# mp3guy/ElasticFusion

Hardware: NVIDIA H100
Metric: frames/sec, full track+fuse+predict (processFrame) (higher is better)
Workload: dtype f32

## Files before the change

elasticfusion_b200/csrc/ef_api.cu:

```cuda
#include <math.h>
#include <stddef.h>
#include <stdio.h>
#include <stdlib.h>
#include <string.h>

#include <new>
#include <utility>
#include <vector>

#include "ef_dmath.cuh"
#include "ef_internal.h"

using namespace ef;

extern "C" void ef_default_config(EfConfig* c, int width, int height, float fx, float fy, float cx, float cy) {
  memset(c, 0, sizeof(*c));
  c->width = width;
  c->height = height;
  c->fx = fx;
  c->fy = fy;
  c->cx = cx;
  c->cy = cy;
  c->time_delta = 200;
  c->count_thresh = 35000;
// ... 23 lines not shown
  if (code > 0) return cudaGetErrorString((cudaError_t)code);
  return "unknown error";
}

static int alloc_odom(EfContext* ctx, OdomDev& od) {
  const EfConfig& c = ctx->cfg;
  memset(&od, 0, sizeof(od));
  od.width = c.width;
  od.height = c.height;
  od.distThres = 0.10f;
  od.angleThres = sinf(20.f * 3.14159254f / 180.f);
  od.sobelScale = (float)(1.0 / pow(2.0, 3));
  od.maxDepthDeltaRGB = 0.07f;
  od.maxDepthRGB = 6.0f;
  od.minGrad[0] = 5;
  od.minGrad[1] = 3;
  od.minGrad[2] = 1;
  for (int i = 0; i < NUM_PYRS; ++i) {
    od.minScale[i] = (float)(pow((double)od.minGrad[i], 2.0) / pow((double)od.sobelScale, 2.0));
    od.rows[i] = c.height >> i;
    od.cols[i] = c.width >> i;
    const size_t n = (size_t)od.rows[i] * od.cols[i];
    CU(ctx_alloc(ctx, &od.depth_tmp[i], n, 0));
    CU(ctx_alloc(ctx, &od.vmap_g_prev[i], 3 * n, 0xff));
    CU(ctx_alloc(ctx, &od.nmap_g_prev[i], 3 * n, 0xff));
    CU(ctx_alloc(ctx, &od.vmap_c_prev[i], 3 * n, 0xff));
    CU(ctx_alloc(ctx, &od.nmap_c_prev[i], 3 * n, 0xff));
    CU(ctx_alloc(ctx, &od.vmap_curr[i], 3 * n, 0xff));
    CU(ctx_alloc(ctx, &od.nmap_curr[i], 3 * n, 0xff));
    CU(ctx_alloc(ctx, &od.lastDepth[i], n, 0xff));
    CU(ctx_alloc(ctx, &od.nextDepth[i], n, 0xff));
    CU(ctx_alloc(ctx, &od.lastImage[i], n, 0));
    CU(ctx_alloc(ctx, &od.nextImage[i], n, 0));
    CU(ctx_alloc(ctx, &od.lastNextImage[i], n, 0));
    CU(ctx_alloc(ctx, &od.dIdx[i], n, 0));
    CU(ctx_alloc(ctx, &od.dIdy[i], n, 0));
    CU(ctx_alloc(ctx, &od.corres[i], n, 0));
  }
  const size_t n0 = (size_t)c.width * c.height;
  CU(ctx_alloc(ctx, &od.vmaps_tmp, 4 * n0, 0));
  CU(ctx_alloc(ctx, &od.gn, 1));
  od.cand_base = reinterpret_cast<const int*>(reinterpret_cast<const char*>(od.gn) + offsetof(GNState, cand_base));
  od.intr0 = reinterpret_cast<const float*>(reinterpret_cast<const char*>(od.gn) + offsetof(GNState, fx));
  od.K_levels = reinterpret_cast<const double*>(reinterpret_cast<const char*>(od.gn) + offsetof(GNState, Kd));
  CU(ctx_alloc(ctx, &od.so3s, 1, 0));
  CU(ctx_alloc(ctx, &od.so3_partials, (size_t)MAX_RED_BLOCKS * PARTIAL_STRIDE, 0));
  CU(ctx_alloc(ctx, &od.so3_counter, 4, 0));
  CU(ctx_alloc(ctx, &od.partials, (size_t)MAX_RED_BLOCKS * PARTIAL_STRIDE, 0));
  CU(ctx_alloc(ctx, &od.partials_rgb, (size_t)MAX_RGB_BLOCKS * 32, 0));
  CU(ctx_alloc(ctx, &od.partials2, (size_t)MAX_RGB_BLOCKS * 32, 0));
  {
    size_t flat = 0;
    for (int i = 0; i < NUM_PYRS; ++i) {
      od.level_start[i] = (int)flat;
      flat += (size_t)od.rows[i] * od.cols[i];
    }
    od.level_start[NUM_PYRS] = (int)flat;
    CU(ctx_alloc(ctx, &od.cand, flat, 0));
    CU(ctx_alloc(ctx, &od.terms, flat, 0));
  }
  CU(ctx_alloc(ctx, &od.partials_i, (size_t)MAX_RED_BLOCKS * 2));
  CU(ctx_alloc(ctx, &od.counter, 4, 0));
  CU(ctx_alloc(ctx, &od.trace, MAX_TRACE, 0));
  GNState g;
  memset(&g, 0, sizeof(g));
  for (int k = 0; k < 16; ++k) g.T_wc[k] = (k % 5 == 0) ? 1.0 : 0.0;
  g.lastICPCount = g.lastRGBCount = g.lastSO3Count = (float)(c.width * c.height);
  g.fx = c.fx;
  g.fy = c.fy;
  g.cx = c.cx;
  g.cy = c.cy;
  for (int lv = 0; lv < NUM_PYRS; ++lv) {
    const int div = 1 << lv;
    const double fx = (double)(c.fx / div), fy = (double)(c.fy / div), cx = (double)(c.cx / div), cy = (double)(c.cy / div);
    const double K[9] = {fx, 0, cx, 0, fy, cy, 0, 0, 1};
    const double ifx = 1.0 / fx, ify = 1.0 / fy;
    const double Ki[9] = {ifx, 0, -cx * ifx, 0, ify, -cy * ify, 0, 0, 1};
    for (int k = 0; k < 9; ++k) {
      g.Kd[lv][k] = K[k];
      g.Kinvd[lv][k] = Ki[k];
    }
  }
  g.break_level = -1;
  g.weighting = 1.0f;
  g.flat_n = od.level_start[NUM_PYRS];
  CU(cudaMemcpyAsync(od.gn, &g, sizeof(g), cudaMemcpyHostToDevice, ctx->stream));
  CU(cudaStreamSynchronize(ctx->stream));
  return 0;
}

static int create_buffers(EfContext* ctx) {
  RC(alloc_odom(ctx, ctx->odom[0]));
  RC(alloc_odom(ctx, ctx->odom[1]));
  const size_t n = (size_t)ctx->cfg.width * ctx->cfg.height;
  Textures& t = ctx->tex;
  memset(&t, 0, sizeof(t));
  CU(ctx_alloc(ctx, &t.rgb, n * 3, 0));
  CU(ctx_alloc(ctx, &t.rgba, n * 4, 0));
  CU(ctx_alloc(ctx, &t.depth_raw, n, 0));
  CU(ctx_alloc(ctx, &t.depth_filtered, n, 0));
  CU(ctx_alloc(ctx, &t.depth_metric, n, 0));
  CU(ctx_alloc(ctx, &t.depth_metric_filtered, n, 0));
  CU(ctx_alloc(ctx, &t.index, n, 0));
  CU(ctx_alloc(ctx, &t.vert_conf, n, 0));
  CU(ctx_alloc(ctx, &t.color_time, n, 0));
  CU(ctx_alloc(ctx, &t.norm_rad, n, 0));
  CU(ctx_alloc(ctx, &t.image, n, 0));
  CU(ctx_alloc(ctx, &t.old_image, n, 0));
  CU(ctx_alloc(ctx, &t.fill_image, n, 0));
  CU(ctx_alloc(ctx, &t.vertex, n, 0));
  CU(ctx_alloc(ctx, &t.normal, n, 0));
  CU(ctx_alloc(ctx, &t.old_vertex, n, 0));
  CU(ctx_alloc(ctx, &t.old_normal, n, 0));
  CU(ctx_alloc(ctx, &t.fill_vertex, n, 0));
  CU(ctx_alloc(ctx, &t.fill_normal, n, 0));
  CU(ctx_alloc(ctx, &t.time, n, 0));
  CU(ctx_alloc(ctx, &t.old_time, n, 0));
  CU(ctx_alloc(ctx, &t.synth_depth, n, 0));
  Lookahead& la = ctx->la;
  memset(&la, 0, sizeof(la));
  CU(ctx_alloc(ctx, &la.rgb, n * 3, 0));
  CU(ctx_alloc(ctx, &la.rgba, n * 4, 0));
  CU(ctx_alloc(ctx, &la.depth_raw, n, 0));
  CU(ctx_alloc(ctx, &la.depth_filtered, n, 0));
  CU(ctx_alloc(ctx, &la.depth_metric, n, 0));
  CU(ctx_alloc(ctx, &la.depth_metric_filtered, n, 0));
  for (int i = 0; i < NUM_PYRS; ++i) {
    const size_t ni = (size_t)ctx->odom[0].rows[i] * ctx->odom[0].cols[i];
    CU(ctx_alloc(ctx, &la.depth_tmp[i], ni, 0));
    CU(ctx_alloc(ctx, &la.vmap_curr[i], 3 * ni, 0xff));
    CU(ctx_alloc(ctx, &la.nmap_curr[i], 3 * ni, 0xff));
    CU(ctx_alloc(ctx, &la.image[i], ni, 0));
  }
  CU(ctx_alloc(ctx, &la.so3s, 1, 0));
  CU(ctx_alloc(ctx, &la.so3_partials, (size_t)MAX_RED_BLOCKS * PARTIAL_STRIDE, 0));
  CU(ctx_alloc(ctx, &la.so3_counter, 4, 0));
  CU(cudaStreamCreateWithFlags(&la.stream, cudaStreamNonBlocking));
  CU(cudaEventCreateWithFlags(&la.ready, cudaEventDisableTiming));
  CU(cudaEventCreateWithFlags(&la.spare_free, cudaEventDisableTiming));
  CU(cudaEventCreateWithFlags(&la.h2d_done, cudaEventDisableTiming));
  CU(cudaEventCreateWithFlags(&la.image_ready, cudaEventDisableTiming));
  CU(cudaEventCreateWithFlags(&la.track_started, cudaEventDisableTiming));
  if (ctx->stage_timing) {
    CU(cudaEventCreate(&la.timing[0]));
    CU(cudaEventCreate(&la.timing[1]));
  }
  CU(cudaMallocHost((void**)&la.pin_rgb, n * 3));
  CU(cudaMallocHost((void**)&la.pin_depth, n * 2));
  RC(alloc_map(ctx));
  CU(cudaMallocHost((void**)&ctx->pin_rgb, n * 3));
  CU(cudaMallocHost((void**)&ctx->pin_depth, n * 2));
  CU(cudaMallocHost((void**)&ctx->pin_small, sizeof(PinStaging)));
  CU(cudaMalloc((void**)&ctx->dev_small, sizeof(DevStaging)));
  CU(cudaEventRecord(la.spare_free, ctx->stream));
  CU(cudaEventRecord(la.h2d_done, la.stream));
  CU(cudaEventRecord(la.image_ready, ctx->stream));
  CU(cudaStreamSynchronize(ctx->stream));
  return 0;
}

extern "C" int ef_create(const EfConfig* cfg, void* stream, EfContext** out) {
  if (!cfg || !out || cfg->width <= 0 || cfg->height <= 0 || cfg->capacity <= 0) return EF_EINVAL;
  if (cfg->reloc) return EF_EINVAL;
  if ((cfg->width >> 2) < 8 || (cfg->height >> 2) < 8) return EF_EINVAL;
  CU(cudaSetDevice(cfg->device));
  EfContext* ctx = new (std::nothrow) EfContext();
  if (!ctx) return EF_ENOMEM;
  ctx->cfg = *cfg;
  ctx->device = cfg->device;
  {
    int sms = 0;
    cudaError_t e = cudaDeviceGetAttribute(&sms, cudaDevAttrMultiProcessorCount, cfg->device);
    ctx->num_sms = sms;
    ctx->own_stream = false;
    if (e == cudaSuccess) {
      if (stream) {
        ctx->stream = (cudaStream_t)stream;
      } else {
        e = cudaStreamCreateWithFlags(&ctx->stream, cudaStreamNonBlocking);
        ctx->own_stream = (e == cudaSuccess);
      }
    }
    if (e != cudaSuccess) {
      delete ctx;
      return (int)e;
    }
  }
  ctx->launches = 0;
  ctx->so3_ready = false;
  {
    const char* e = getenv("EF_NO_PDL");
    ctx->pdl = !(e && e[0] == '1');
    ctx->plain_next = false;
    ctx->maps_dirty[0] = ctx->maps_dirty[1] = true;
    e = getenv("EF_VISIBLE_LIST");
    ctx->visible_list = !(e && e[0] == '0');
    ctx->vis_pending = false;
    e = getenv("EF_GN_CLUSTER");
    ctx->gn_cluster = odom_cluster_size(e ? atoi(e) : 16);
    e = getenv("EF_GN_CLUSTER_LEVELS");
    ctx->gn_cluster_levels = e ? atoi(e) : 1;
    if (ctx->gn_cluster_levels < 0) ctx->gn_cluster_levels = 0;
    if (ctx->gn_cluster_levels > NUM_PYRS) ctx->gn_cluster_levels = NUM_PYRS;
    e = getenv("EF_STAGE_TIMING");
    ctx->stage_timing = (e && e[0] == '1');
    ctx->stage_n = 0;
    if (ctx->stage_timing)
      for (int i = 0; i < 16; ++i) cudaEventCreate(&ctx->stage_ev[i]);
    e = getenv("EF_LA_AFTER_TRACK");
    ctx->la_after_track = !(e && e[0] == '0');
  }
  ctx->tick = 1;
  for (int k = 0; k < 16; ++k) ctx->T_wc[k] = (k % 5 == 0) ? 1.0 : 0.0;
  ctx->rgb_only = false;
  ctx->icp_weight = cfg->icp_weight;
  ctx->pyramid = true;
  ctx->fast_odom = cfg->fast_odom != 0;
  ctx->so3 = cfg->so3 != 0;
  ctx->frame_to_frame_rgb = cfg->frame_to_frame_rgb != 0;
  ctx->confidence = cfg->confidence;
  ctx->depth_cutoff = cfg->depth_cutoff;
  ctx->max_depth_processed = 20.0f;
  ctx->host_count = 0;
  ctx->frame_open = false;

  if (int rc = create_buffers(ctx)) {
    ef_destroy(ctx);
    return rc;
  }
  *out = ctx;
  return 0;
}

extern "C" int ef_destroy(EfContext* ctx) {
  if (!ctx) return EF_EINVAL;
  cudaSetDevice(ctx->device);
  cudaStreamSynchronize(ctx->stream);
  if (ctx->la.stream) {
    cudaStreamSynchronize(ctx->la.stream);
    cudaStreamDestroy(ctx->la.stream);
  }
  if (ctx->la.ready) cudaEventDestroy(ctx->la.ready);
  if (ctx->la.spare_free) cudaEventDestroy(ctx->la.spare_free);
  if (ctx->la.h2d_done) cudaEventDestroy(ctx->la.h2d_done);
  if (ctx->la.image_ready) cudaEventDestroy(ctx->la.image_ready);
  if (ctx->la.track_started) cudaEventDestroy(ctx->la.track_started);
  for (cudaEvent_t ev : ctx->la.timing)
    if (ev) cudaEventDestroy(ev);
  if (ctx->la.pin_rgb) cudaFreeHost(ctx->la.pin_rgb);
  if (ctx->la.pin_depth) cudaFreeHost(ctx->la.pin_depth);
  map_free_host(ctx);
  deform_free(ctx);
  ctx->arena.release();
  if (ctx->pin_rgb) cudaFreeHost(ctx->pin_rgb);
  if (ctx->pin_depth) cudaFreeHost(ctx->pin_depth);
  if (ctx->pin_small) cudaFreeHost(ctx->pin_small);
  if (ctx->dev_small) cudaFree(ctx->dev_small);
  if (ctx->own_stream) cudaStreamDestroy(ctx->stream);
  delete ctx;
  return 0;
}

extern "C" void* ef_stream(EfContext* ctx) { return ctx ? (void*)ctx->stream : nullptr; }
extern "C" int ef_sync(EfContext* ctx) {
  if (!ctx) return EF_EINVAL;
  CU(cudaStreamSynchronize(ctx->stream));
  CU(cudaStreamSynchronize(ctx->la.stream));
  return 0;
}
extern "C" int ef_launch_count(EfContext* ctx, int64_t* n) {
  if (!ctx || !n) return EF_EINVAL;
  *n = ctx->launches;
  return 0;
}

extern "C" int ef_buffer(EfContext* ctx, int32_t id, int32_t level, void** dev_ptr, size_t* bytes) {
  if (!ctx) return EF_EINVAL;
  const size_t n = (size_t)ctx->cfg.width * ctx->cfg.height;
  void* p = nullptr;
  size_t b = 0;
  Textures& t = ctx->tex;
  if (id < 40) {
    switch (id) {
      case EF_BUF_RGB: p = t.rgb; b = n * 3; break;
      case EF_BUF_RGBA: p = t.rgba; b = n * 4; break;
      case EF_BUF_DEPTH_RAW: p = t.depth_raw; b = n * 2; break;
      case EF_BUF_DEPTH_FILTERED: p = t.depth_filtered; b = n * 2; break;
      case EF_BUF_DEPTH_METRIC: p = t.depth_metric; b = n * 4; break;
      case EF_BUF_DEPTH_METRIC_FILTERED: p = t.depth_metric_filtered; b = n * 4; break;
      case EF_BUF_INDEX: p = t.index; b = n * 4; break;
      case EF_BUF_VERT_CONF: p = t.vert_conf; b = n * 16; break;
      case EF_BUF_COLOR_TIME: p = t.color_time; b = n * 16; break;
      case EF_BUF_NORM_RAD: p = t.norm_rad; b = n * 16; break;
      case EF_BUF_IMAGE: p = t.image; b = n * 4; break;
      case EF_BUF_VERTEX: p = t.vertex; b = n * 16; break;
      case EF_BUF_NORMAL: p = t.normal; b = n * 16; break;
      case EF_BUF_TIME: p = t.time; b = n * 2; break;
      case EF_BUF_OLD_IMAGE: p = t.old_image; b = n * 4; break;
      case EF_BUF_OLD_VERTEX: p = t.old_vertex; b = n * 16; break;
      case EF_BUF_OLD_NORMAL: p = t.old_normal; b = n * 16; break;
      case EF_BUF_OLD_TIME: p = t.old_time; b = n * 2; break;
      case EF_BUF_SYNTH_DEPTH: p = t.synth_depth; b = n * 4; break;
      case EF_BUF_FILL_IMAGE: p = t.fill_image; b = n * 4; break;
      case EF_BUF_FILL_VERTEX: p = t.fill_vertex; b = n * 16; break;
      case EF_BUF_FILL_NORMAL: p = t.fill_normal; b = n * 16; break;
      default: return EF_EINVAL;
// ... 535 lines not shown
    ef_stage(ctx, 10);
  }
  if (ctx->tick == 1) RC(map_update_pose_async(ctx, nullptr));
  RC(predict_async(ctx));
  ef_stage(ctx, 11);
  ctx->tick++;
  ctx->frame_open = false;
  return 0;
}

extern "C" int ef_process_frame_device(EfContext* ctx, const uint8_t* rgb_dev, const uint16_t* depth_dev, int64_t timestamp,
                                       float weight_multiplier, const double* in_T_wc) {
  (void)timestamp;
  if (!ctx || ((rgb_dev == nullptr) != (depth_dev == nullptr))) return EF_EINVAL;
  RC(frame_begin_device(ctx, rgb_dev, depth_dev, weight_multiplier, in_T_wc));
  return frame_end_device(ctx, 0, false);
}

static int stage_host_frame(EfContext* ctx, const uint8_t* rgb, const uint16_t* depth) {
  const size_t n = (size_t)ctx->cfg.width * ctx->cfg.height;
  CU(cudaStreamSynchronize(ctx->stream));
  memcpy(ctx->pin_rgb, rgb, n * 3);
  memcpy(ctx->pin_depth, depth, n * 2);
  CU(cudaMemcpyAsync(ctx->tex.rgb, ctx->pin_rgb, n * 3, cudaMemcpyHostToDevice, ctx->stream));
  CU(cudaMemcpyAsync(ctx->tex.depth_raw, ctx->pin_depth, n * 2, cudaMemcpyHostToDevice, ctx->stream));
  return 0;
}

extern "C" int ef_process_frame_begin(EfContext* ctx, const uint8_t* rgb, const uint16_t* depth, int64_t timestamp, float weight_multiplier,
                                      const double* in_T_wc) {
  (void)timestamp;
  if (!ctx || !rgb || !depth) return EF_EINVAL;
  if (ctx->la.pending || ctx->frame_open) return EF_ESTATE;
  RC(stage_host_frame(ctx, rgb, depth));
  RC(frame_begin_device(ctx, ctx->tex.rgb, ctx->tex.depth_raw, weight_multiplier, in_T_wc));
  return ef_finish_frame(ctx);
}

extern "C" int ef_process_frame_end(EfContext* ctx, const double* T_wc_override, const float* graph_nodes16, int32_t n_nodes, int32_t fern_accepted) {
  if (!ctx || n_nodes < 0 || (n_nodes > 0 && !graph_nodes16)) return EF_EINVAL;
  if (!ctx->frame_open) return EF_ESTATE;
  if (T_wc_override) {
    RC(ef_set_pose(ctx, T_wc_override));
    RC(map_update_pose_async(ctx, nullptr));
  }
  RC(map_set_graph(ctx, graph_nodes16, n_nodes));
  RC(frame_end_device(ctx, n_nodes, fern_accepted != 0));
  return ef_finish_frame(ctx);
}

extern "C" int ef_local_loop_result(EfContext* ctx, EfLoopResult* out, double* src3, double* dst3, int32_t* times, int32_t max_constraints,
                                    int32_t* n_out) {
  if (!ctx || !out || max_constraints < 0) return EF_EINVAL;
  const MapDev& m = ctx->map;
  LoopDev h;
  CU(cudaMemcpyAsync(&h, m.loop, sizeof(h), cudaMemcpyDeviceToHost, ctx->stream));
  CU(cudaStreamSynchronize(ctx->stream));
  out->ran = h.ran;
  out->accepted = h.accepted;
  out->n_constraints = h.n_constraints;
  out->lastICPError = h.lastICPError;
  out->lastICPCount = h.lastICPCount;
  memcpy(out->cov_diag, h.cov_diag, sizeof(h.cov_diag));
  memcpy(out->T_wc_est, h.T_wc_est, sizeof(h.T_wc_est));
  int n = h.n_constraints < max_constraints ? h.n_constraints : max_constraints;
  if (n > m.loop_capacity) n = m.loop_capacity;
  if (n_out) *n_out = n;
  if (n > 0) {
    if (src3) CU(cudaMemcpyAsync(src3, m.loop_src, sizeof(double) * 3 * n, cudaMemcpyDeviceToHost, ctx->stream));
    if (dst3) CU(cudaMemcpyAsync(dst3, m.loop_dst, sizeof(double) * 3 * n, cudaMemcpyDeviceToHost, ctx->stream));
    if (times) CU(cudaMemcpyAsync(times, m.loop_times, sizeof(int) * n, cudaMemcpyDeviceToHost, ctx->stream));
    CU(cudaStreamSynchronize(ctx->stream));
  }
  return 0;
}

extern "C" int ef_deform_solve(EfContext* ctx, const double* node_pos3, const int32_t* node_times, int32_t n_nodes, const double* src3,
                               const double* dst3, const int32_t* src_times, const int32_t* dst_times, int32_t n_constraints, int32_t pin,
                               int32_t last_deform_time, float* nodes16, double* rt12, int32_t* cons_nodes4, double* cons_weights4,
                               EfDeformResult* out) {
  if (!ctx || !out || !node_pos3 || !node_times || !src3 || !dst3 || !src_times || (pin && !dst_times)) return EF_EINVAL;
  if (n_nodes < 5 || n_nodes >= MAX_GRAPH_NODES || n_constraints < 1 || last_deform_time < 0) return EF_EINVAL;
  for (int i = 0; i < n_nodes; ++i)
    if (node_times[i] < 0 || (i > 0 && node_times[i] < node_times[i - 1])) return EF_EINVAL;
  const int m = pin ? 2 * n_constraints : n_constraints;
  std::vector<double> s(3 * (size_t)m), d(3 * (size_t)m);
  std::vector<int32_t> t(m);
  for (int i = 0, o = 0; i < n_constraints; ++i) {
    if (src_times[i] < 0 || (pin && dst_times[i] < 0)) return EF_EINVAL;
    memcpy(&s[3 * o], src3 + 3 * i, sizeof(double) * 3);
    memcpy(&d[3 * o], dst3 + 3 * i, sizeof(double) * 3);
    t[o++] = src_times[i];
    if (pin) {
      memcpy(&s[3 * o], dst3 + 3 * i, sizeof(double) * 3);
      memcpy(&d[3 * o], dst3 + 3 * i, sizeof(double) * 3);
      t[o++] = dst_times[i];
    }
  }
  CU(cudaSetDevice(ctx->device));
  return deform_solve(ctx, node_pos3, node_times, n_nodes, s.data(), d.data(), t.data(), m, last_deform_time, nodes16, rt12,
                      cons_nodes4, cons_weights4, out);
}

extern "C" int ef_join_lookahead(EfContext* ctx) {
  if (!ctx) return EF_EINVAL;
  if (ctx->la.pending) CU(cudaStreamWaitEvent(ctx->stream, ctx->la.ready, 0));
  return 0;
}

extern "C" int ef_finish_frame(EfContext* ctx) {
  if (!ctx) return EF_EINVAL;
  PinStaging* s = ctx->pin_small;
  CU(cudaMemcpyAsync(s->finish_T_wc, ctx->odom[0].gn->T_wc, sizeof(double) * 16, cudaMemcpyDeviceToHost, ctx->stream));
  CU(cudaMemcpyAsync(&s->finish_count, ctx->map.count, 4, cudaMemcpyDeviceToHost, ctx->stream));
  CU(cudaStreamSynchronize(ctx->stream));
  memcpy(ctx->T_wc, s->finish_T_wc, sizeof(double) * 16);
  ctx->host_count = s->finish_count;
  return 0;
}

extern "C" int ef_process_frame(EfContext* ctx, const uint8_t* rgb, const uint16_t* depth, int64_t timestamp, float weight_multiplier,
                                const double* in_T_wc) {
  if (!ctx || ((rgb == nullptr) != (depth == nullptr))) return EF_EINVAL;
  if (!rgb) {
    RC(ef_process_frame_device(ctx, nullptr, nullptr, timestamp, weight_multiplier, in_T_wc));
    return ef_finish_frame(ctx);
  }
  if (ctx->la.pending) return EF_ESTATE;
  RC(stage_host_frame(ctx, rgb, depth));
  RC(ef_process_frame_device(ctx, ctx->tex.rgb, ctx->tex.depth_raw, timestamp, weight_multiplier, in_T_wc));
  return ef_finish_frame(ctx);
}

extern "C" int ef_debug_stage_ms(EfContext* ctx, float* out) {
  if (!ctx || !ctx->stage_timing) return 0;
  cudaStreamSynchronize(ctx->stream);
  int prev = -1;
  for (int i = 0; i < 16; ++i) {
    out[i] = 0.f;
    if (!(ctx->stage_n >> i & 1)) continue;
    if (prev >= 0) cudaEventElapsedTime(&out[i], ctx->stage_ev[prev], ctx->stage_ev[i]);
    prev = i;
  }
  return 12;
}
extern "C" int ef_debug_lookahead_ms(EfContext* ctx, float* out2) {
  if (!ctx || !out2 || !ctx->stage_timing || !(ctx->stage_n & 1)) return 0;
  if (cudaStreamSynchronize(ctx->la.stream) != cudaSuccess) return 0;
  for (int i = 0; i < 2; ++i)
    if (cudaEventElapsedTime(&out2[i], ctx->stage_ev[0], ctx->la.timing[i]) != cudaSuccess) return 0;
  return 2;
}
extern "C" void* ef_debug_gn(EfContext* ctx, int which) { return ctx ? (void*)ctx->odom[which].gn : nullptr; }
extern "C" int ef_debug_gn_size() { return (int)sizeof(GNState); }
extern "C" int ef_debug_dbg_offset() { return (int)offsetof(GNState, dbg); }
```

elasticfusion_b200/csrc/ef_internal.h:

```cpp
#pragma once
#include <cuda_runtime.h>
#include <stdint.h>

#include <vector>

#include "../../include/efusion_b200.h"

namespace ef {

constexpr int NUM_PYRS = 3;
constexpr int RED_THREADS = 256;
constexpr int MAX_RED_BLOCKS = 1184;
constexpr int PARTIAL_STRIDE = 64;
constexpr int MAX_TRACE = 48;
constexpr int MAX_RGB_BLOCKS = 160;

struct DataTerm {
  short zero_x, zero_y;
  short one_x, one_y;
  float diff;
  int valid;
};

struct GNState {
  double T_wc[16];
  float lastICPError, lastICPCount, lastRGBError, lastRGBCount, lastSO3Error, lastSO3Count;
  double lastA[36], lastb[6];

  float Rprev[9], tprev[3], Rprev_inv[9];
  float Rcurr[9], tcurr[3];
  float Mcp[9], tcp[3];
  double resultRt[16];
  int break_level;

  float krkinv[9], kt[3];
  float sigmaVal;
  int rgbSize, sigma;

  float sum_icp[32], sum_rgb[32];
  int sum_res[2];
  unsigned int res_acc[2];

  int rgbOnly, icp, rgb, so3;
  float icpWeight;
  float fx, fy, cx, cy;
  double Kd[NUM_PYRS][9], Kinvd[NUM_PYRS][9];
  int trace_n;
  int cand_base[NUM_PYRS + 1];
  int flat_n;
  float rgbErrBuf[2];
  float weighting;
  long long dbg[40];
};

constexpr int SO3_MAX_ITER = 10;
struct So3State {
  double resultR[9], lastResultR[9];
  float R_lr[9];
  float imageBasis[9], kinv[9], krlr[9];
  float so3_lastError, so3_lastCount;
  int so3_done;
  float sum_so3[12];
  float lastSO3Error, lastSO3Count;
  int trace_n;
  EfSolveTrace trace[SO3_MAX_ITER];
};

struct MapPose {
  float pose[16];
  float t_inv[16];
};

struct OdomDev {
  int width, height;
  int rows[NUM_PYRS], cols[NUM_PYRS];
  float distThres, angleThres;
  float sobelScale, maxDepthDeltaRGB, maxDepthRGB;
  float minGrad[NUM_PYRS];
  float minScale[NUM_PYRS];

  uint16_t* depth_tmp[NUM_PYRS];
  float* vmaps_tmp;
  float *vmap_g_prev[NUM_PYRS], *nmap_g_prev[NUM_PYRS], *vmap_curr[NUM_PYRS], *nmap_curr[NUM_PYRS];
  float *vmap_c_prev[NUM_PYRS], *nmap_c_prev[NUM_PYRS];
  float *lastDepth[NUM_PYRS], *nextDepth[NUM_PYRS];
  uint8_t *lastImage[NUM_PYRS], *nextImage[NUM_PYRS], *lastNextImage[NUM_PYRS];
  int16_t *dIdx[NUM_PYRS], *dIdy[NUM_PYRS];
  DataTerm* corres[NUM_PYRS];
  int4* cand;
  const int* cand_base;
  const float* intr0;
  const double* K_levels;
  int4* terms;
  int level_start[NUM_PYRS + 1];

  GNState* gn;
  So3State* so3s;
  float* so3_partials;
  unsigned int* so3_counter;
  float* partials;
  double* partials2;
  float* partials_rgb;
  int* partials_i;
  unsigned int* counter;
  EfSolveTrace* trace;
};

constexpr int MAX_GRAPH_NODES = 1024;

struct LoopDev {
  int ran, accepted, n_constraints;
  float lastICPError, lastICPCount;
  double cov_diag[6];
  double T_wc_est[16];
};

inline int loop_constraint_capacity(int width, int height) { return (width / 20) * (height / 20); }

struct MapDev {
  int rows, cols;
  float cx, cy, fx, fy;
  int capacity;
  float4 *pos_conf, *color_time, *norm_rad;
  int* count;
  float4 *new_pos, *new_col, *new_nr;
  int* new_count;
  uint32_t* assoc_id;
  uint32_t* pending;
  unsigned long long* zbuf;
  int* scan_tile_state;
  unsigned int* scan_counter;
  uint32_t* vis_list;
  int* vis_count;
  unsigned int* clean_ctl;
  uint32_t* keep_mask;
  uint8_t* flags;
  float4 *fb_raw[3], *fb_filt[3];
  int* fb_count;
  MapPose* pose;
  int* dense_flag;
  int* tick;
  float* nodes;
  LoopDev* loop;
  int loop_capacity;
  double *loop_src, *loop_dst;
  int* loop_times;
};

struct Textures {
  uint8_t* rgb;
  uint8_t* rgba;
  uint16_t* depth_raw;
  uint16_t* depth_filtered;
  float* depth_metric;
  float* depth_metric_filtered;
  uint32_t* index;
  float4 *vert_conf, *color_time, *norm_rad;
  uchar4 *image, *old_image, *fill_image;
  float4 *vertex, *normal, *old_vertex, *old_normal, *fill_vertex, *fill_normal;
  uint16_t *time, *old_time;
  float* synth_depth;
};

struct Lookahead {
  cudaStream_t stream;
  cudaEvent_t ready;
  cudaEvent_t spare_free;
  cudaEvent_t h2d_done;
  cudaEvent_t image_ready;
  cudaEvent_t track_started;
  bool track_marked;
  cudaEvent_t timing[2];
  bool pending;
  uint8_t *rgb, *rgba;
  uint16_t *depth_raw, *depth_filtered;
  float *depth_metric, *depth_metric_filtered;
  uint16_t* depth_tmp[NUM_PYRS];
  float *vmap_curr[NUM_PYRS], *nmap_curr[NUM_PYRS];
  uint8_t* image[NUM_PYRS];
  So3State* so3s;
  float* so3_partials;
  unsigned int* so3_counter;
  bool so3_ready;
  uint8_t* pin_rgb;
  uint16_t* pin_depth;
};

struct Arena {
  std::vector<void*> blocks;
  template <typename T>
  cudaError_t alloc(T** p, size_t n) {
    void* q = nullptr;
    cudaError_t e = cudaMalloc(&q, n * sizeof(T) + 256);
    if (e != cudaSuccess) return e;
    blocks.push_back(q);
    *p = (T*)q;
    return cudaSuccess;
  }
  void release() {
    for (void* p : blocks) cudaFree(p);
    blocks.clear();
  }
};

struct PinStaging {
  float icp_inputs[36];
  double map_pose[16];
  float weighting;
  double T_wc[16];
  double finish_T_wc[16];
  int finish_count;
};
struct DevStaging {
  double map_pose[16];
  double T_wc[16];
};
static_assert(sizeof(PinStaging) <= 65536 && sizeof(DevStaging) <= 65536, "staging blocks stay within 64 KiB");

}

struct EfContext {
  EfConfig cfg;
  int device;
  int num_sms;
  cudaStream_t stream;
  bool own_stream;
  int64_t launches;
  bool stage_timing;
  cudaEvent_t stage_ev[16];
  int stage_n;
  bool pdl;
  bool vis_pending;
  bool visible_list;
  int gn_cluster;
  int gn_cluster_levels;
  bool la_after_track;
  bool plain_next;
  bool maps_dirty[2];

  ef::OdomDev odom[2];
  ef::MapDev map;
  ef::Textures tex;
  ef::Lookahead la;
  bool so3_ready;

  int tick;
  double T_wc[16];
  bool rgb_only;
  float icp_weight;
  bool pyramid, fast_odom, so3, frame_to_frame_rgb;
  float confidence, depth_cutoff, max_depth_processed;
  int host_count;
  bool frame_open;

  uint8_t* pin_rgb;
  uint16_t* pin_depth;
  ef::PinStaging* pin_small;
  ef::DevStaging* dev_small;
  void* map_host;
  void* deform;
  ef::Arena arena;
};

#define CU(x)                                  \
  do {                                         \
    cudaError_t e__ = (x);                     \
    if (e__ != cudaSuccess) return (int)e__;   \
  } while (0)
#define RC(x)              \
  do {                     \
    int rc__ = (x);        \
    if (rc__) return rc__; \
  } while (0)
#define CHECK_LAST() CU(cudaGetLastError())

namespace ef {
template <typename T>
inline cudaError_t ctx_alloc(EfContext* ctx, T** p, size_t n, int fill = -1) {
  cudaError_t e = ctx->arena.alloc(p, n);
  if (e != cudaSuccess || fill < 0) return e;
  return cudaMemsetAsync(*p, fill, n * sizeof(T), ctx->stream);
}
}

inline void ef_stage(EfContext* ctx, int i) {
  if (ctx->stage_timing) {
    cudaEventRecord(ctx->stage_ev[i], ctx->stream);
    if (i == 0) ctx->stage_n = 0;
    ctx->stage_n |= 1 << i;
  }
}
inline cudaLaunchAttribute cluster_attr(int cluster) {
  cudaLaunchAttribute a;
  a.id = cudaLaunchAttributeClusterDimension;
  a.val.clusterDim.x = cluster;
  a.val.clusterDim.y = 1;
  a.val.clusterDim.z = 1;
  return a;
}
template <typename... KArgs, typename... Args>
inline void ef_launch(EfContext* ctx, void (*kernel)(KArgs...), dim3 grid, dim3 block, size_t smem, int cluster, Args&&... args) {
  cudaLaunchConfig_t cfg = {};
  cfg.gridDim = grid;
  cfg.blockDim = block;
  cfg.dynamicSmemBytes = smem;
  cfg.stream = ctx->stream;
  cudaLaunchAttribute attr[2];
  int n = 0;
  if (cluster > 0) attr[n++] = cluster_attr(cluster);
  if (ctx->pdl && !ctx->plain_next) {
    attr[n].id = cudaLaunchAttributeProgrammaticStreamSerialization;
    attr[n++].val.programmaticStreamSerializationAllowed = 1;
  }
  cfg.attrs = attr;
  cfg.numAttrs = n;
  ctx->plain_next = false;
  cudaLaunchKernelEx(&cfg, kernel, static_cast<KArgs>(args)...);
  ctx->launches++;
}
#define EF_LAUNCH(ctx, kernel, grid, block, smem, ...) ef_launch((ctx), kernel, dim3(grid), dim3(block), (smem), 0, __VA_ARGS__)
#define EF_PLAIN_NEXT(ctx) ((ctx)->plain_next = true)

inline int wave_blocks(const EfContext* ctx, size_t n, int per_sm = 8, int threads = 256) {
  size_t b = (n + threads - 1) / threads, cap = (size_t)ctx->num_sms * per_sm;
  return (int)(b < cap ? (b ? b : 1) : cap);
}

namespace ef {
int odom_init_icp_depth(EfContext* ctx, int which, const uint16_t* depth_dev, float cutoff);
int odom_init_icp_pred(EfContext* ctx, int which, const float* vtx4, const float* nrm4);
int odom_init_icp_model(EfContext* ctx, int which, const float* vtx4, const float* nrm4, bool with_global = true);
int odom_populate(EfContext* ctx, int which, const uint8_t* rgba, float** destDepths, uint8_t** destImages, bool with_depth,
                  bool with_image = true);
int map_select_model_inputs(EfContext* ctx);
int launch_sobel(EfContext* ctx, int which);

int odom_cluster_size(int want);
int odom_so3_async(EfContext* ctx, int which);
int odom_track_async(EfContext* ctx, int which, bool rgbOnly, float icpWeight, bool pyramid, bool fastOdom, bool so3);
int odom_finish_async(EfContext* ctx, int which, float weightMultiplier, bool have_track);
int odom_set_pose_async(EfContext* ctx, int which, const double* T_dev);
int launch_se3_step_raw(EfContext* ctx, int which, int level, bool do_icp, bool do_rgb, float sigma);
int launch_rgb_residual_raw(EfContext* ctx, int which, int level);
int launch_icp_dense_only(EfContext* ctx, int which, int level);
int launch_so3_raw(EfContext* ctx, int which);

int preprocess_depth(EfContext* ctx, const uint16_t* raw, float cutoff, uint16_t* filtered, float* metric, float* metric_filtered);
int rgb_to_rgba(EfContext* ctx, const uint8_t* rgb, uint8_t* rgba);

int alloc_map(EfContext* ctx);
void map_free_host(EfContext* ctx);
int run_scan(EfContext* ctx, const uint8_t* flags, const int* n_a, const int* n_b, size_t max_items, int* offsets, int* total);
void scan_scratch(EfContext* ctx, uint8_t** flags, int** offsets);
int map_initialise_async(EfContext* ctx);
int map_update_pose_async(EfContext* ctx, const double* T_host_or_null);
int map_predict_indices_async(EfContext* ctx, int time_or_neg, float max_depth, int time_delta, int vis_mode = 0);
int map_fuse_async(EfContext* ctx, int time_or_neg, float max_depth, float weighting_or_neg);
int map_clean_async(EfContext* ctx, int time_or_neg, float conf_threshold, int time_delta, float max_depth, int n_nodes = 0, bool is_fern = false);
int map_set_graph(EfContext* ctx, const float* nodes16, int n_nodes);
int map_raycast_async(EfContext* ctx, float max_depth, float conf_threshold, int time, int max_time, int time_delta, int mode);
int map_fill_in_async(EfContext* ctx, bool passthrough_geometry, bool passthrough_image);
int map_dense_enough_async(EfContext* ctx);
int map_loop_constraints_async(EfContext* ctx, int count_thresh, float err_thresh, float cov_thresh);
int map_loop_reset_async(EfContext* ctx);
int odom_copy_pose_async(EfContext* ctx, int dst, int src);
int map_download(EfContext* ctx, const float4* a, const float4* b, const float4* c, int n, float* out);
int map_upload(EfContext* ctx, const float* in, int n);
int map_upload_range(EfContext* ctx, const float* in, int first, int n);
int map_resize_to_host(EfContext* ctx, const void* src_dev, int elem, int factor, void* host_out);

int deform_solve(EfContext* ctx, const double* node_pos3, const int32_t* node_times, int n, const double* src3, const double* dst3,
                 const int32_t* src_times, int m, int last_deform_time, float* nodes16_host, double* rt12_host,
                 int32_t* cons_nodes4, double* cons_weights4, EfDeformResult* out);
void deform_free(EfContext* ctx);
}
```

elasticfusion_b200/csrc/ef_preprocess.cu:

```cuda
#include "ef_device.cuh"
#include "ef_internal.h"

using namespace ef;

namespace {
constexpr int TILE_X = 32, TILE_Y = 8, R = 6;
constexpr int SM_W = TILE_X + 2 * R, SM_H = TILE_Y + 2 * R;
}

__global__ void __launch_bounds__(TILE_X* TILE_Y) k_preprocess_depth(const uint16_t* __restrict__ depth, int rows, int cols, float maxD,
                                                                      uint16_t* __restrict__ filtered, float* __restrict__ metric,
                                                                      float* __restrict__ metric_filtered) {
  pdl_enter();
  __shared__ float tile[SM_H][SM_W + 1];
  const int x0 = blockIdx.x * TILE_X - R, y0 = blockIdx.y * TILE_Y - R;
  for (int i = threadIdx.y * TILE_X + threadIdx.x; i < SM_W * SM_H; i += TILE_X * TILE_Y) {
    const int ty = i / SM_W, tx = i - ty * SM_W;
    const int gx = x0 + tx, gy = y0 + ty;
    tile[ty][tx] = (gx >= 0 && gy >= 0 && gx < cols && gy < rows) ? (float)depth[(size_t)gy * cols + gx] : 0.f;
  }
  __syncthreads();
  const int x = blockIdx.x * TILE_X + threadIdx.x, y = blockIdx.y * TILE_Y + threadIdx.y;
  if (x >= cols || y >= rows) return;
  const size_t p = (size_t)y * cols + x;
  const unsigned int hi = (unsigned int)(maxD * 1000.0f);
  const unsigned int value = depth[p];
  const bool gated = (value > hi || value < 300U);
  if (metric) metric[p] = gated ? 0.f : (float)value / 1000.0f;
  unsigned int out = 0;
  if (!gated) {
    const float sigma_space2_inv_half = 0.024691358f;
    const float sigma_color2_inv_half = 0.000555556f;
    const int D = R * 2 + 1;
    const int tx = min(x - D / 2 + D, cols);
    const int ty = min(y - D / 2 + D, rows);
    float sum1 = 0, sum2 = 0;
    const float fv = (float)value;
    for (int cy = max(y - D / 2, 0); cy < ty; ++cy) {
      const float dy = (float)y - (float)cy;
      const float* trow = tile[cy - y0];
      for (int cx = max(x - D / 2, 0); cx < tx; ++cx) {
        const float tmp = trow[cx - x0];
        const float dx = (float)x - (float)cx;
        const float space2 = dx * dx + dy * dy;
        const float color2 = (fv - tmp) * (fv - tmp);
        const float weight = expf(-(space2 * sigma_space2_inv_half + color2 * sigma_color2_inv_half));
        sum1 += tmp * weight;
        sum2 += weight;
      }
    }
    out = (unsigned int)roundf(sum1 / sum2);
  }
  if (filtered) filtered[p] = (uint16_t)out;
  if (metric_filtered) metric_filtered[p] = (out > hi || out < 300U) ? 0.f : (float)out / 1000.0f;
}

__global__ void k_rgb_to_rgba(const uint8_t* __restrict__ rgb, uchar4* __restrict__ rgba, size_t n) {
  pdl_enter();
  for (size_t p = (size_t)blockIdx.x * blockDim.x + threadIdx.x; p < n; p += (size_t)gridDim.x * blockDim.x)
    rgba[p] = make_uchar4(rgb[p * 3 + 0], rgb[p * 3 + 1], rgb[p * 3 + 2], 255);
}

namespace ef {
int preprocess_depth(EfContext* ctx, const uint16_t* raw, float cutoff, uint16_t* filtered, float* metric, float* metric_filtered) {
  const int rows = ctx->cfg.height, cols = ctx->cfg.width;
  dim3 grid((cols + TILE_X - 1) / TILE_X, (rows + TILE_Y - 1) / TILE_Y), block(TILE_X, TILE_Y);
  EF_LAUNCH(ctx, k_preprocess_depth, grid, block, 0, raw, rows, cols, cutoff, filtered, metric, metric_filtered);
  CHECK_LAST();
  return 0;
}
int rgb_to_rgba(EfContext* ctx, const uint8_t* rgb, uint8_t* rgba) {
  const size_t n = (size_t)ctx->cfg.height * ctx->cfg.width;
  EF_LAUNCH(ctx, k_rgb_to_rgba, wave_blocks(ctx, n), 256, 0, rgb, (uchar4*)rgba, n);
  CHECK_LAST();
  return 0;
}
}
```

Before: 1350.

## Replace bilateral expf with precomputed weight table and taller output tiles

Precomputes the bilateral filter weights once at init into a table indexed by spatial distance class and integer depth difference, so the per-pixel 13x13 window does a table load instead of expf. Out-of-image neighbours are set to a large negative sentinel whose weight falls to zero, which replaces the clamped loop bounds and lets the window loop unroll fully. Each block now computes four rows per thread so the halo rows are loaded once for more outputs. The table is checked at init to confirm weights beyond the row length are exactly zero. The change adds a gather-style table read per tap and depends on that check for exactness.

```diff
diff --git a/elasticfusion_b200/csrc/ef_api.cu b/elasticfusion_b200/csrc/ef_api.cu
--- a/elasticfusion_b200/csrc/ef_api.cu
+++ b/elasticfusion_b200/csrc/ef_api.cu
@@ -199,6 +199,7 @@
   CU(cudaMallocHost((void**)&ctx->pin_depth, n * 2));
   CU(cudaMallocHost((void**)&ctx->pin_small, sizeof(PinStaging)));
   CU(cudaMalloc((void**)&ctx->dev_small, sizeof(DevStaging)));
+  RC(bilateral_table_init(ctx));
   CU(cudaEventRecord(la.spare_free, ctx->stream));
   CU(cudaEventRecord(la.h2d_done, la.stream));
   CU(cudaEventRecord(la.image_ready, ctx->stream));
@@ -1040,5 +1041,10 @@
   return 2;
 }
 extern "C" void* ef_debug_gn(EfContext* ctx, int which) { return ctx ? (void*)ctx->odom[which].gn : nullptr; }
+extern "C" const float* ef_debug_bilateral_table(EfContext* ctx, int* classes, int* row) {
+  if (classes) *classes = BILAT_CLASSES;
+  if (row) *row = BILAT_ROW;
+  return ctx ? ctx->bilateral_w : nullptr;
+}
 extern "C" int ef_debug_gn_size() { return (int)sizeof(GNState); }
 extern "C" int ef_debug_dbg_offset() { return (int)offsetof(GNState, dbg); }
diff --git a/elasticfusion_b200/csrc/ef_internal.h b/elasticfusion_b200/csrc/ef_internal.h
--- a/elasticfusion_b200/csrc/ef_internal.h
+++ b/elasticfusion_b200/csrc/ef_internal.h
@@ -14,6 +14,8 @@
 constexpr int PARTIAL_STRIDE = 64;
 constexpr int MAX_TRACE = 48;
 constexpr int MAX_RGB_BLOCKS = 160;
+constexpr int BILAT_CLASSES = 27;
+constexpr int BILAT_ROW = 436;
 
 struct DataTerm {
   short zero_x, zero_y;
@@ -210,10 +212,12 @@
   double T_wc[16];
   double finish_T_wc[16];
   int finish_count;
+  int table_ok;
 };
 struct DevStaging {
   double map_pose[16];
   double T_wc[16];
+  int table_ok;
 };
 static_assert(sizeof(PinStaging) <= 65536 && sizeof(DevStaging) <= 65536, "staging blocks stay within 64 KiB");
 
@@ -242,6 +246,7 @@
   ef::MapDev map;
   ef::Textures tex;
   ef::Lookahead la;
+  float* bilateral_w;
   bool so3_ready;
 
   int tick;
@@ -345,6 +350,7 @@
 int launch_icp_dense_only(EfContext* ctx, int which, int level);
 int launch_so3_raw(EfContext* ctx, int which);
 
+int bilateral_table_init(EfContext* ctx);
 int preprocess_depth(EfContext* ctx, const uint16_t* raw, float cutoff, uint16_t* filtered, float* metric, float* metric_filtered);
 int rgb_to_rgba(EfContext* ctx, const uint8_t* rgb, uint8_t* rgba);
 
diff --git a/elasticfusion_b200/csrc/ef_preprocess.cu b/elasticfusion_b200/csrc/ef_preprocess.cu
--- a/elasticfusion_b200/csrc/ef_preprocess.cu
+++ b/elasticfusion_b200/csrc/ef_preprocess.cu
@@ -4,55 +4,103 @@
 using namespace ef;
 
 namespace {
-constexpr int TILE_X = 32, TILE_Y = 8, R = 6;
-constexpr int SM_W = TILE_X + 2 * R, SM_H = TILE_Y + 2 * R;
+constexpr int TILE_X = 32, TILE_Y = 8, PX_Y = 4, R = 6;
+constexpr int OUT_Y = TILE_Y * PX_Y;
+constexpr int SM_W = TILE_X + 2 * R, SM_H = OUT_Y + 2 * R;
+constexpr float SIGMA_SPACE2_INV_HALF = 0.024691358f, SIGMA_COLOR2_INV_HALF = 0.000555556f;
+constexpr float OUTSIDE = -65536.f;
+
+__host__ __device__ constexpr int space_class(int dx, int dy) {
+  const int s = dx * dx + dy * dy;
+  int c = 0;
+  for (int v = 0; v < s; ++v) {
+    bool hit = false;
+    for (int a = 0; a <= R; ++a)
+      for (int b = 0; b <= R; ++b) hit = hit || (a * a + b * b == v);
+    c += hit;
+  }
+  return c;
+}
+static_assert(space_class(R, R) + 1 == BILAT_CLASSES, "BILAT_CLASSES = distinct dx^2 + dy^2 of the 13x13 window");
+
+__device__ __forceinline__ float bilateral_weight(float space2, float color2) {
+  return expf(-(space2 * SIGMA_SPACE2_INV_HALF + color2 * SIGMA_COLOR2_INV_HALF));
+}
+}
+
+__global__ void k_bilateral_table(float* __restrict__ W, int* __restrict__ ok) {
+  pdl_enter();
+  __shared__ int first_zero, nonzero_after;
+  const int c = blockIdx.x;
+  int s2 = 0;
+  for (int dy = 0; dy <= R; ++dy)
+    for (int dx = 0; dx <= R; ++dx)
+      if (space_class(dx, dy) == c) s2 = dx * dx + dy * dy;
+  const float space2 = (float)s2;
+  if (threadIdx.x == 0) {
+    first_zero = 65536;
+    nonzero_after = 0;
+  }
+  __syncthreads();
+  for (int d = threadIdx.x; d < 65536; d += blockDim.x) {
+    const float fd = (float)d;
+    const float w = bilateral_weight(space2, fd * fd);
+    if (w == 0.f) atomicMin(&first_zero, d);
+    if (d < BILAT_ROW) W[c * BILAT_ROW + d] = w;
+  }
+  __syncthreads();
+  for (int d = first_zero + threadIdx.x; d < 65536; d += blockDim.x) {
+    const float fd = (float)d;
+    if (bilateral_weight(space2, fd * fd) != 0.f) nonzero_after = 1;
+  }
+  __syncthreads();
+  if (threadIdx.x == 0 && (nonzero_after || first_zero > BILAT_ROW - 1)) *ok = 0;
 }
 
 __global__ void __launch_bounds__(TILE_X* TILE_Y) k_preprocess_depth(const uint16_t* __restrict__ depth, int rows, int cols, float maxD,
-                                                                      uint16_t* __restrict__ filtered, float* __restrict__ metric,
-                                                                      float* __restrict__ metric_filtered) {
+                                                                      const float* __restrict__ table, uint16_t* __restrict__ filtered,
+                                                                      float* __restrict__ metric, float* __restrict__ metric_filtered) {
   pdl_enter();
   __shared__ float tile[SM_H][SM_W + 1];
-  const int x0 = blockIdx.x * TILE_X - R, y0 = blockIdx.y * TILE_Y - R;
-  for (int i = threadIdx.y * TILE_X + threadIdx.x; i < SM_W * SM_H; i += TILE_X * TILE_Y) {
+  const int tid = threadIdx.y * TILE_X + threadIdx.x;
+  const int x0 = blockIdx.x * TILE_X - R, y0 = blockIdx.y * OUT_Y - R;
+  for (int i = tid; i < SM_W * SM_H; i += TILE_X * TILE_Y) {
     const int ty = i / SM_W, tx = i - ty * SM_W;
     const int gx = x0 + tx, gy = y0 + ty;
-    tile[ty][tx] = (gx >= 0 && gy >= 0 && gx < cols && gy < rows) ? (float)depth[(size_t)gy * cols + gx] : 0.f;
+    tile[ty][tx] = (gx >= 0 && gy >= 0 && gx < cols && gy < rows) ? (float)depth[(size_t)gy * cols + gx] : OUTSIDE;
   }
   __syncthreads();
-  const int x = blockIdx.x * TILE_X + threadIdx.x, y = blockIdx.y * TILE_Y + threadIdx.y;
-  if (x >= cols || y >= rows) return;
-  const size_t p = (size_t)y * cols + x;
+  const int x = blockIdx.x * TILE_X + threadIdx.x;
+  if (x >= cols) return;
   const unsigned int hi = (unsigned int)(maxD * 1000.0f);
-  const unsigned int value = depth[p];
-  const bool gated = (value > hi || value < 300U);
-  if (metric) metric[p] = gated ? 0.f : (float)value / 1000.0f;
-  unsigned int out = 0;
-  if (!gated) {
-    const float sigma_space2_inv_half = 0.024691358f;
-    const float sigma_color2_inv_half = 0.000555556f;
-    const int D = R * 2 + 1;
-    const int tx = min(x - D / 2 + D, cols);
-    const int ty = min(y - D / 2 + D, rows);
-    float sum1 = 0, sum2 = 0;
-    const float fv = (float)value;
-    for (int cy = max(y - D / 2, 0); cy < ty; ++cy) {
-      const float dy = (float)y - (float)cy;
-      const float* trow = tile[cy - y0];
-      for (int cx = max(x - D / 2, 0); cx < tx; ++cx) {
-        const float tmp = trow[cx - x0];
-        const float dx = (float)x - (float)cx;
-        const float space2 = dx * dx + dy * dy;
-        const float color2 = (fv - tmp) * (fv - tmp);
-        const float weight = expf(-(space2 * sigma_space2_inv_half + color2 * sigma_color2_inv_half));
-        sum1 += tmp * weight;
-        sum2 += weight;
-      }
+#pragma unroll 1
+  for (int k = 0; k < PX_Y; ++k) {
+    const int y = blockIdx.y * OUT_Y + k * TILE_Y + threadIdx.y;
+    if (y >= rows) return;
+    const size_t p = (size_t)y * cols + x;
+    const unsigned int value = depth[p];
+    const bool gated = (value > hi || value < 300U);
+    if (metric) metric[p] = gated ? 0.f : (float)value / 1000.0f;
+    unsigned int out = 0;
+    if (!gated) {
+      float sum1 = 0, sum2 = 0;
+      const float fv = (float)value;
+      const float* trow = &tile[y - y0 - R][x - x0 - R];
+#pragma unroll
+      for (int dy = -R; dy <= R; ++dy)
+#pragma unroll
+        for (int dx = -R; dx <= R; ++dx) {
+          const float tmp = trow[(dy + R) * (SM_W + 1) + dx + R];
+          const int d = __float_as_int(fabsf(fv - tmp) + 8388608.f) - 0x4B000000;
+          const float weight = __ldg(&table[space_class(dx, dy) * BILAT_ROW + min(d, BILAT_ROW - 1)]);
+          sum1 += tmp * weight;
+          sum2 += weight;
+        }
+      out = (unsigned int)roundf(sum1 / sum2);
     }
-    out = (unsigned int)roundf(sum1 / sum2);
+    if (filtered) filtered[p] = (uint16_t)out;
+    if (metric_filtered) metric_filtered[p] = (out > hi || out < 300U) ? 0.f : (float)out / 1000.0f;
   }
-  if (filtered) filtered[p] = (uint16_t)out;
-  if (metric_filtered) metric_filtered[p] = (out > hi || out < 300U) ? 0.f : (float)out / 1000.0f;
 }
 
 __global__ void k_rgb_to_rgba(const uint8_t* __restrict__ rgb, uchar4* __restrict__ rgba, size_t n) {
@@ -62,10 +110,23 @@
 }
 
 namespace ef {
+int bilateral_table_init(EfContext* ctx) {
+  CU(ctx_alloc(ctx, &ctx->bilateral_w, (size_t)BILAT_CLASSES * BILAT_ROW));
+  int* ok = &ctx->dev_small->table_ok;
+  ctx->pin_small->table_ok = 1;
+  CU(cudaMemcpyAsync(ok, &ctx->pin_small->table_ok, sizeof(int), cudaMemcpyHostToDevice, ctx->stream));
+  EF_LAUNCH(ctx, k_bilateral_table, BILAT_CLASSES, 1024, 0, ctx->bilateral_w, ok);
+  CHECK_LAST();
+  CU(cudaMemcpyAsync(&ctx->pin_small->table_ok, ok, sizeof(int), cudaMemcpyDeviceToHost, ctx->stream));
+  CU(cudaStreamSynchronize(ctx->stream));
+  return ctx->pin_small->table_ok ? 0 : EF_ESTATE;
+}
+
 int preprocess_depth(EfContext* ctx, const uint16_t* raw, float cutoff, uint16_t* filtered, float* metric, float* metric_filtered) {
   const int rows = ctx->cfg.height, cols = ctx->cfg.width;
-  dim3 grid((cols + TILE_X - 1) / TILE_X, (rows + TILE_Y - 1) / TILE_Y), block(TILE_X, TILE_Y);
-  EF_LAUNCH(ctx, k_preprocess_depth, grid, block, 0, raw, rows, cols, cutoff, filtered, metric, metric_filtered);
+  dim3 grid((cols + TILE_X - 1) / TILE_X, (rows + OUT_Y - 1) / OUT_Y), block(TILE_X, TILE_Y);
+  EF_LAUNCH(ctx, k_preprocess_depth, grid, block, 0, raw, rows, cols, cutoff, (const float*)ctx->bilateral_w, filtered, metric,
+            metric_filtered);
   CHECK_LAST();
   return 0;
 }
```

Result: no change. 1363, median of 6 (+0.9%).
